# rgl-epfl/large-steps-pytorch

Measured on AMD Instinct MI355X. Metric: from_differential_solves_per_sec, higher is better.
Workload: dtype f32; 1 GPU; cfg4_plane1m: 1000x1000 plane, V=1000000, nnz(M)=6992002, M=I+50*L_uniform, u=M v, k=3, factor once (not timed), re-solve timed; method=nested-dissection, device=AMD Radeon Graphics

## Files before the change

### large-steps-pytorch_amd/csrc/direct.hip

```cpp
#include "common.h"
#include <vector>
#include <chrono>
#include <algorithm>
#include <atomic>
#include <string.h>
#include <memory>
#include <mutex>

namespace ls {

struct alignas(64) Tile {
    int store;
    int row0, s, b, own_start, bnd_off, front_off;
    int leaf;
    int pfront_off, cix;
    int forward;
    int arity;
    long long finv_off, w_off;
};

static_assert(sizeof(Tile) == 64, "Tile layout");
__device__ __forceinline__ Tile load_tile(const Tile* __restrict__ tiles, int idx) {
    const int lane = threadIdx.x & 63;
    const int w = lane < 16 ? reinterpret_cast<const int*>(tiles)[(size_t)idx * 16 + lane] : 0;
// ... 902 lines not shown
                    it.s = n.s; it.b = n.b; it.own_start = n.own_start; it.bnd_off = n.bnd_off; it.front_off = n.front_off;
                    it.pfront_off = n.pfront_off; it.cix = n.cix; it.flags = n.flags | (lv > root ? NODE_UPC : 0); it.finv_off = n.finv_off; it.w_off = n.w_off;
                    it.spb_off = n.spb_off; it.sps_off = n.sps_off; it.nparts = 1;
                    if (n.flags & NODE_SPARSE) {
                        items.push_back(it);
                        leaf_need = std::max(leaf_need, std::max(tri_cap, (4 * n.b + 3) & ~3) + 256);
                        continue;
                    }
                    if (n.s == 0 && n.b == 0) continue;
                    const int rows = up ? n.b : n.s, L = up ? ((n.s + 3) & ~3) : ((n.s + 3) & ~3) + ((n.b + 3) & ~3);
                    int nparts = 1;
                    if (!sparse && base < waves) nparts = std::max(1, std::min(waves / std::max(base, 1), L / 16));
                    for (int r = 0; r < std::max(rows, 1); r += WAVE)
                        for (int pt = 0; pt < nparts; ++pt) {
                            it.row0 = r; it.r0 = (int)((int64_t)(L / 4) * pt / nparts) * 4; it.r1 = (int)((int64_t)(L / 4) * (pt + 1) / nparts) * 4;
                            it.part = pt; it.nparts = nparts;
                            items.push_back(it);
                            vec_need = std::max(vec_need, 4 * (it.r1 - it.r0 + 32));
                        }
                    if (nparts > 1) { if (up) g.up_split |= 1u << ph; else g.down_split |= 1u << ph; }
                }
                if (all_sparse) { if (up) g.up_leaf |= 1u << ph; else g.down_leaf |= 1u << ph; }
                else if (sparse) return 0;
                const int n_items = (int)items.size() - off[ph];
                if (((up ? g.up_split : g.down_split) >> ph) & 1u) pbuf_need = std::max(pbuf_need, div_up(n_items, waves) * 256);
            }
            off[H] = (int)items.size();
        }
    }
    vec_floats = (vec_need + 3) & ~3;
    return (size_t)std::max(vec_floats + pbuf_need, leaf_need);
}


static size_t direct_tier_lds(int levels, int arity, const int* s, const int* b, const int* own_start, int tier_levels, bool sparse_leaves, int waves) {
    std::vector<int64_t> level_off((size_t)levels + 1);
    int64_t cnt = 1, off = 1;
    for (int lv = 0; lv <= levels; ++lv) { level_off[lv] = off; off += cnt; cnt *= arity; }
    const int64_t n_nodes = level_off[levels] - 1;
    std::vector<NodeD> nd((size_t)n_nodes + 1);
    memset(nd.data(), 0, nd.size() * sizeof(NodeD));
    const int root = levels - tier_levels;
    for (int lv = root; lv < levels; ++lv)
        for (int64_t i = level_off[lv]; i < level_off[lv + 1]; ++i) {
            NodeD& q = nd[(size_t)i];
            q.s = s[i]; q.b = b[i]; q.own_start = own_start[i];
            const bool sparse = sparse_leaves && lv == levels - 1 && q.s >= 1;
            q.flags = (lv + 1 >= levels ? NODE_LEAF : 0) | (sparse ? NODE_SPARSE : NODE_QUAD);
        }
    std::vector<TierItem> items;
    std::vector<TierWG> wgs;
    int vec = 0, tri = 0;
    const size_t region = plan_tier(nd, level_off, levels, arity, root, 0, level_off[root + 1] - level_off[root], items, wgs, vec, tri, waves);
    return region ? ((region + 3) & ~(size_t)3) * sizeof(float) * waves : 0;
}

bool direct_tier_fits(int levels, int arity, const int* s, const int* b, const int* own_start, int tier_levels, bool sparse_leaves, int waves) {
    if (tier_levels <= 0) return true;
    if (tier_levels > levels || tier_levels > TIER_MAX_H) return false;
    const size_t bytes = direct_tier_lds(levels, arity, s, b, own_start, tier_levels, sparse_leaves, waves);
    return bytes && bytes <= (size_t)(waves == TIER_WAVES_FULL ? TIER_LDS_FULL : TIER_LDS);
}

extern "C" int ls_direct_tier_lds_bytes(int levels, int arity, const int32_t* h_s, const int32_t* h_b, const int32_t* h_own_start, int tier_levels,
                                        int sparse_leaves, int waves, size_t* h_bytes) {
    LS_REQUIRE(h_s && h_b && h_own_start && h_bytes && levels >= 1 && levels <= 30 && (arity == 2 || arity == 4 || arity == 8) &&
               tier_levels >= 1 && tier_levels <= levels && tier_levels <= TIER_MAX_H && (waves == TIER_WAVES || waves == TIER_WAVES_WIDE || waves == TIER_WAVES_FULL),
               LS_E_INVALID, "ls_direct_tier_lds_bytes: bad argument (1 <= tier_levels <= min(levels, %d); waves 4, 8 or 16)", TIER_MAX_H);
    *h_bytes = direct_tier_lds(levels, arity, h_s, h_b, h_own_start, tier_levels, sparse_leaves != 0, waves);
    return LS_OK;
}

bool direct_tier_full16(int64_t V, int arity, int levels, int tier_levels, int shard_count, int tier_waves) {
    if (tier_waves == TIER_WAVES_FULL) return tier_levels >= 2;
    if (tier_waves == TIER_WAVES || tier_waves == TIER_WAVES_WIDE) return false;
    return shard_count <= 1 && arity == 4 && levels >= 8 && V >= 800000 && tier_levels == levels - 4 && tier_levels <= TIER_MAX_H;
}


namespace {
struct CreatePlan {
    int levels = 0, arity = 0, cut = 0;
    int64_t sub_lo = 0, sub_hi = 1;
    std::vector<int64_t> level_off;
    std::vector<NodeD> nd;
    std::vector<int> parent;
    std::vector<unsigned char> mask;
    std::vector<TierItem> items;
    std::vector<TierWG> wgs;
    std::vector<int> pull;
    std::vector<Tile> tiles;
    std::vector<PackedTile> ptiles;
    int64_t span(int from, int to) const { int64_t s = 1; for (int t = from; t < to; ++t) s *= arity; return s; }
    bool active(int64_t i, int lv) const {
        if (lv < cut) return true;
        int64_t q = i - level_off[lv];
        for (int t = cut; t < lv; ++t) q /= arity;
        return q >= sub_lo && q < sub_hi;
    }
};

int read_nodes(const ls_direct_arrays* A, CreatePlan& T, ls_direct* d) {
    const int levels = T.levels, n_nodes = d->n_nodes;
    T.nd.assign((size_t)n_nodes + 1, NodeD());
    T.parent.assign((size_t)n_nodes + 1, 0);
    d->lvl_up.assign((size_t)levels, 0); d->lvl_down.assign((size_t)levels, 0); d->lvl_rows.assign((size_t)levels, 0); d->lvl_bnd.assign((size_t)levels, 0);
    int64_t fe = 0, fe_up = 0, fe_down = 0;
// ... 27 lines not shown
    }
    fe += 2 * A->n_sp_ent + A->n_sp_ptr;
    fe_up += A->n_sp_ent + A->n_sp_ptr / 2; fe_down += A->n_sp_ent + A->n_sp_ptr - A->n_sp_ptr / 2;
    d->lvl_up[(size_t)levels - 1] += A->n_sp_ent + A->n_sp_ptr / 2; d->lvl_down[(size_t)levels - 1] += A->n_sp_ent + A->n_sp_ptr - A->n_sp_ptr / 2;
    d->factor_entries = fe; d->words_up = fe_up; d->words_down = fe_down;
    {
        const double mb = 4e-6 * (double)fe;
        d->nt_rule[0] = d->nt_levels = mb > 256.0;
        d->nt_rule[1] = d->nt_tier = mb > 400.0;
    }
    for (int lv = 1; lv < levels; ++lv)
        for (int64_t i = T.level_off[lv]; i < T.level_off[lv + 1]; ++i) {
            const NodeD &n = T.nd[i], &p = T.nd[T.parent[i]];
            for (int k = 0; k < n.b; ++k) {
                const int pp = A->h_ppos[n.bnd_off + k];
                if (pp < 0 || pp >= p.s + p.b) {
                    set_error("ls_direct_create: ppos out of range at node %lld", (long long)i);
                    return LS_E_INVALID;
                }
                T.mask[(size_t)p.front_off + pp] |= (unsigned char)(1u << n.cix);
            }
        }
    return LS_OK;
}

int choose_tier(CreatePlan& T, const int32_t* h_ppos, int tier_waves, const NdEnv& env, ls_direct* d) {
    const int levels = T.levels;
    int root = levels;
    for (int lv = levels - 1; lv >= 0; --lv) {
        bool tiered = false, plain = false;
        for (int64_t i = T.level_off[lv]; i < T.level_off[lv + 1]; ++i) {
            if (T.nd[i].s == 0 && T.nd[i].b == 0) continue;
            if (T.nd[i].flags & (NODE_SPARSE | NODE_QUAD)) tiered = true; else plain = true;
        }
        if (tiered && plain) { set_error("ls_direct_create: level %d mixes tier-layout and plain nodes", lv); return LS_E_INVALID; }
        if (plain) break;
        if (tiered && root != lv + 1) { set_error("ls_direct_create: tier-layout levels must be the deepest ones"); return LS_E_INVALID; }
        if (tiered) root = lv;
    }
    for (int lv = 0; lv < root; ++lv)
        for (int64_t i = T.level_off[lv]; i < T.level_off[lv + 1]; ++i)
            if (T.nd[i].flags & (NODE_SPARSE | NODE_QUAD)) { set_error("ls_direct_create: tier-layout node above the tier"); return LS_E_INVALID; }
    d->tier_root = levels;
    if (root == levels) return LS_OK;
    const int H = levels - root;
    if (T.cut > root) { set_error("ls_direct_create: %d ranks need a cut below the tier's root level (tree too small)", d->shard_count); return LS_E_INVALID; }
    const int64_t span = T.span(T.cut, root), q_lo = T.sub_lo * span, q_hi = T.sub_hi * span;
    size_t region = 0;
    auto take_if_fits = [&](int waves, int budget) {
        std::vector<TierItem> items;
        std::vector<TierWG> wgs;
        int vec = 0, tri = 0;
        const size_t r = plan_tier(T.nd, T.level_off, levels, T.arity, root, q_lo, q_hi, items, wgs, vec, tri, waves);
        if (!r || ((r + 3) & ~(size_t)3) * sizeof(float) * waves > (size_t)budget) return;
        T.items.swap(items); T.wgs.swap(wgs); d->tier_vec = vec; d->tier_tri = tri; region = r; d->tier_waves = waves;
    };
    if (H <= TIER_MAX_H && direct_tier_full16(d->V, T.arity, levels, H, d->shard_count, tier_waves > 0 ? tier_waves : env.tier_waves.value_or(0)))
        take_if_fits(TIER_WAVES_FULL, TIER_LDS_FULL);
    if (!region) {
        region = H <= TIER_MAX_H ? plan_tier(T.nd, T.level_off, levels, T.arity, root, q_lo, q_hi, T.items, T.wgs, d->tier_vec, d->tier_tri) : 0;
        if (!region || region * sizeof(float) * TIER_WAVES > TIER_LDS) {
            set_error("ls_direct_create: a tier of %d levels does not fit the kernel (LDS per wave: %zu floats)", H, region);
            return LS_E_WORKSPACE;
        }
        if (H >= 2 && (int)T.wgs.size() <= 768 && (tier_waves > 0 ? tier_waves : env.tier_waves.value_or(TIER_WAVES_WIDE)) == TIER_WAVES_WIDE)
            take_if_fits(TIER_WAVES_WIDE, TIER_LDS_WIDE);
    }
    d->tier_root = root; d->tier_phases = H; d->tier_wgs = (int)T.wgs.size(); d->tier_region = (int)((region + 3) & ~(size_t)3);
    d->pull_base = T.nd[T.level_off[root]].front_off;
    T.pull.assign((size_t)std::max<int64_t>(0, T.nd[T.level_off[levels - 1]].front_off - d->pull_base) * T.arity, -1);
    for (int lv = root + 1; lv < levels; ++lv)
        for (int64_t i = T.level_off[lv]; i < T.level_off[lv + 1]; ++i) {
            const NodeD& n = T.nd[i];
            for (int k = 0; k < n.b; ++k) T.pull[(size_t)(n.pfront_off - d->pull_base + h_ppos[n.bnd_off + k]) * T.arity + n.cix] = n.bnd_off + k;
        }
    return LS_OK;
}

size_t plan_level(CreatePlan& T, int lv, int long_up, const NdEnv& env, int kmax, LevelPlan& p) {
    std::vector<Tile>& tiles = T.tiles;
    int64_t a0 = T.level_off[lv], a1 = T.level_off[lv + 1];
    if (lv >= T.cut) { const int64_t span = T.span(T.cut, lv); a0 = T.level_off[lv] + T.sub_lo * span; a1 = T.level_off[lv] + T.sub_hi * span; }
    auto tile_of = [&](int64_t i, int r, int forward) {
        const NodeD& n = T.nd[i];
        Tile t;
        t.store = 0; t.row0 = r; t.s = n.s; t.b = n.b; t.own_start = n.own_start; t.bnd_off = n.bnd_off; t.front_off = n.front_off;
        t.leaf = lv + 1 >= T.levels; t.pfront_off = n.pfront_off; t.cix = n.cix;
        t.forward = forward; t.arity = T.arity; t.finv_off = n.finv_off; t.w_off = n.w_off;
        return t;
    };
    int red_up = 0, red_down = 0;
    for (int64_t i = a0; i < a1; ++i) {
        p.s_cap = std::max(p.s_cap, T.nd[i].s); p.b_cap = std::max(p.b_cap, T.nd[i].b);
        red_up = std::max(red_up, T.nd[i].s); red_down = std::max(red_down, T.nd[i].s + T.nd[i].b);
    }
    p.up_b = red_up >= long_up; p.down_b = red_down >= env.long_red;
    const int up_bw = std::min(ND_BW, red_up >= 1400 ? 8 : 4), down_bw = std::min(ND_BW, red_down >= 1400 ? 8 : 4);
    p.up_nw = p.up_b ? up_bw : pick_nw(red_up, 32); p.down_nw = p.down_b ? down_bw : pick_nw(red_down, env.steps);
    int64_t rows_up = 0, rows_down = 0;
    for (int64_t i = a0; i < a1; ++i) { rows_up += T.nd[i].b; rows_down += T.nd[i].s; }
    auto pick_chunks = [&](int64_t rows, int bw) {
        int c = 4;
        while (c > 1 && rows / (ND_ROWS * bw * c) < 500) --c;
        return c;
    };
    p.up_chunks = pick_chunks(rows_up, up_bw);
    p.down_chunks = pick_chunks(rows_down, down_bw);
    const int up_rows = p.up_b ? ND_ROWS * up_bw * p.up_chunks : WAVE, down_rows = p.down_b ? ND_ROWS * down_bw * p.down_chunks : WAVE;
    const size_t up_s_bytes = ((size_t)p.s_cap * p.b_cap + (size_t)p.s_cap * kmax) * sizeof(float);
    p.up_s = p.b_cap <= 256 && p.s_cap <= 256 && up_s_bytes <= 40 * 1024 && !env.no_small;
    if (p.up_s) { p.up_b = 0; p.up_nw = std::max(1, div_up(p.b_cap, WAVE)); }
    p.up_p = !env.no_pack && p.b_cap <= WAVE && p.s_cap <= 256 && lv > 0;
    p.down_p = !env.no_pack && p.s_cap <= WAVE / 2;
    auto pack_level = [&](bool up_sweep, int& first, int& count, int& lds_rows_s, int& lds_rows_b) {
// ... 218 lines not shown
#define LS_OPTIN(KK)                                                                                                                \
        (const void*)k_nd_up<KK, false>, (const void*)k_nd_down<KK, false>, (const void*)k_nd_up_b<KK, false>,                      \
        (const void*)k_nd_down_b<KK, false>, (const void*)k_nd_up<KK, true>, (const void*)k_nd_down<KK, true>,                      \
        (const void*)k_nd_up_b<KK, true>, (const void*)k_nd_down_b<KK, true>, (const void*)k_nd_up_s<KK>,
        LS_OPTIN(1) LS_OPTIN(2) LS_OPTIN(3) LS_OPTIN(4)
#undef LS_OPTIN
#define LS_OPTIN(KK)                                                                                                                \
        (const void*)k_nd_tier<KK, true, TIER_WAVES, false>, (const void*)k_nd_tier<KK, false, TIER_WAVES, false>,                  \
        (const void*)k_nd_tier<KK, true, TIER_WAVES, true>, (const void*)k_nd_tier<KK, false, TIER_WAVES, true>,                    \
        (const void*)k_nd_tier<KK, true, TIER_WAVES_WIDE, false>, (const void*)k_nd_tier<KK, false, TIER_WAVES_WIDE, false>,        \
        (const void*)k_nd_tier<KK, true, TIER_WAVES_FULL, false>, (const void*)k_nd_tier<KK, false, TIER_WAVES_FULL, false>,        \
        (const void*)k_nd_tier<KK, true, TIER_WAVES_FULL, true>, (const void*)k_nd_tier<KK, false, TIER_WAVES_FULL, true>,
        LS_OPTIN(1) LS_OPTIN(2) LS_OPTIN(3) LS_OPTIN(4)
#undef LS_OPTIN
    };
    for (const void* k : kernels) (void)hipFuncSetAttribute(k, hipFuncAttributeMaxDynamicSharedMemorySize, LDS_OPTIN);
    lap("kernel attributes set");
    *out = d.release();
    return LS_OK;
}

extern "C" int ls_direct_destroy(ls_direct* d) {
    if (!d) return LS_OK;
    DeviceGuard g(d->device);
    if (d->busy) (void)hipEventDestroy(d->busy);
    if (!d->tables.empty()) (void)hipDeviceSynchronize();
    for (const auto& t : d->tables)
        if (!ls::pool_give(d->device, t.first, t.second)) (void)hipFree(t.first);
    ls::refactor_state_free(d->refac);
    for (hipEvent_t e : d->ev) (void)hipEventDestroy(e);
#ifdef LS_TIER_STAMPS
    if (d->stamps) (void)hipFree(d->stamps);
#endif
    for (hipEvent_t e : d->lev) (void)hipEventDestroy(e);
    delete d;
    return LS_OK;
}

template <int K>
static int direct_solve_k(ls_direct* d, const float* b, float* x, hipStream_t st, int part, float* exchange) {
    const int top = d->tier_root - 1;
    TierArgs ta;
    ta.items = d->d_items; ta.wgs = d->d_wgs; ta.perm = d->perm; ta.mask = d->mask; ta.ppos = d->ppos;
    ta.pull = d->pull ? d->pull - (size_t)d->pull_base * d->arity : nullptr; ta.push_ptr = d->push_ptr; ta.push_tgt = d->push_tgt; ta.u4 = d->u4; ta.d4 = d->d4; ta.tri = d->tri;
    ta.sp_ptr = d->sp_ptr; ta.sp_ent = d->sp_ent; ta.bprime = d->bp; ta.braw = d->braw; ta.slots = d->slots; ta.xb = d->xb;
    ta.arity = d->arity; ta.phases = d->tier_phases; ta.region_floats = d->tier_region; ta.vec_floats = d->tier_vec;
    ta.upper_lo = d->upper_lo; ta.upper_hi = (int)d->V;
#ifdef LS_TIER_STAMPS
    const size_t stamp_n = (size_t)d->tier_wgs * d->tier_waves * TIER_STAMP_SLOTS;
    if (d->profile == 2 && !d->stamps && stamp_n) LS_HIP(hipMalloc((void**)&d->stamps, 2 * stamp_n * sizeof(long long)));
    if (d->profile == 2 && d->stamps) LS_HIP(hipMemsetAsync(d->stamps, 0, 2 * stamp_n * sizeof(long long), st));
    ta.stamps = d->profile == 2 ? d->stamps : nullptr;
#endif
    const size_t tier_lds = (size_t)d->tier_region * d->tier_waves * sizeof(float);
    const bool nt_tier = d->nt_tier && d->tier_waves != TIER_WAVES_WIDE, nt = d->nt_levels;
    int n_mark = 0;
    auto mark = [&](int lo, int hi, int sweep) -> hipError_t {
        if (d->profile != 3) return hipSuccess;
        while ((int)d->lev.size() <= n_mark + 1) { hipEvent_t e; const hipError_t r = hipEventCreate(&e); if (r != hipSuccess) return r; d->lev.push_back(e); }
        if ((int)d->lmeta.size() <= n_mark) d->lmeta.resize((size_t)n_mark + 1);
        d->lmeta[(size_t)n_mark] = {lo, hi, sweep};
        return hipEventRecord(d->lev[(size_t)n_mark++], st);
    };
    auto mark_end = [&]() -> hipError_t {
        if (d->profile != 3) return hipSuccess;
        hipError_t r = hipEventRecord(d->lev[(size_t)n_mark], st);
        if (r == hipSuccess) r = hipStreamSynchronize(st);
        d->launch_ms.assign((size_t)n_mark, 0.0);
        d->lmeta.resize((size_t)n_mark);
        for (int i = 0; i < n_mark && r == hipSuccess; ++i) { float ms = 0; r = hipEventElapsedTime(&ms, d->lev[(size_t)i], d->lev[(size_t)i + 1]); d->launch_ms[(size_t)i] = ms; }
        return r;
    };
    const size_t exch_off = (size_t)d->exch_f0 * d->arity * K, exch_n = (size_t)(d->exch_f1 - d->exch_f0) * d->arity * K;
    if (part != 1) {
    if (d->profile) LS_HIP(hipEventRecord(d->ev[0], st));
    if (part == 0 && exch_n) LS_HIP(hipMemsetAsync(d->slots + exch_off, 0, exch_n * sizeof(float), st));
    if (d->tier_wgs) {
        LS_HIP(mark(d->tier_root, d->levels - 1, 0));
        if (d->tier_waves == TIER_WAVES_FULL && nt_tier) hipLaunchKernelGGL((k_nd_tier<K, true, TIER_WAVES_FULL, true>), dim3(d->tier_wgs), dim3(WAVE * TIER_WAVES_FULL), tier_lds, st, ta, b, x, d->tier_tri);
        else if (d->tier_waves == TIER_WAVES_FULL) hipLaunchKernelGGL((k_nd_tier<K, true, TIER_WAVES_FULL, false>), dim3(d->tier_wgs), dim3(WAVE * TIER_WAVES_FULL), tier_lds, st, ta, b, x, d->tier_tri);
        else if (d->tier_waves == TIER_WAVES_WIDE) hipLaunchKernelGGL((k_nd_tier<K, true, TIER_WAVES_WIDE, false>), dim3(d->tier_wgs), dim3(WAVE * TIER_WAVES_WIDE), tier_lds, st, ta, b, x, d->tier_tri);
        else if (nt_tier) hipLaunchKernelGGL((k_nd_tier<K, true, TIER_WAVES, true>), dim3(d->tier_wgs), dim3(WAVE * TIER_WAVES), tier_lds, st, ta, b, x, d->tier_tri);
        else hipLaunchKernelGGL((k_nd_tier<K, true, TIER_WAVES, false>), dim3(d->tier_wgs), dim3(WAVE * TIER_WAVES), tier_lds, st, ta, b, x, d->tier_tri);
    }
    }
    if (part == 1 && exch_n && exchange != d->slots + exch_off)
        LS_HIP(hipMemcpyAsync(d->slots + exch_off, exchange, exch_n * sizeof(float), hipMemcpyDeviceToDevice, st));
    const int* up_perm = d->tier_wgs ? nullptr : d->perm;
    const float* up_b = d->tier_wgs ? d->braw : b;
    const bool fuse_root = top >= 0 && !d->plan[0].down_p;
    const RootFill rf = fuse_root ? RootFill{up_perm, d->mask, d->slots, up_b} : RootFill{nullptr, nullptr, nullptr, nullptr};
    for (int lv = (part == 1 ? std::min(top, d->cut - 1) : top); lv >= (part == 0 ? d->cut : 0); --lv) {
        const LevelPlan& p = d->plan[lv];
        if (!(p.up_p ? p.up_p_tiles : p.up_tiles)) continue;
        if (lv == 0 && fuse_root) continue;
        LS_HIP(mark(lv, lv, 0));
        if (p.up_p)
            hipLaunchKernelGGL(k_nd_up_p<K>, dim3(p.up_p_tiles), dim3(WAVE), (size_t)std::max(p.up_p_lds, 1) * K * sizeof(float), st,
                               d->ptiles + p.up_p_first, up_perm, d->mask, d->ppos, d->wf, up_b, d->bp, d->slots);
        else if (p.up_s)
            hipLaunchKernelGGL(k_nd_up_s<K>, dim3(p.up_tiles), dim3(WAVE * p.up_nw), ((size_t)p.s_cap * p.b_cap + (size_t)p.s_cap * K) * sizeof(float), st,
                               d->tiles + p.up_first, up_perm, d->mask, d->ppos, d->wf, up_b, d->bp, d->slots, p.s_cap, p.b_cap);
        else if (p.up_b)
            hipLaunchKernelGGL((nt ? k_nd_up_b<K, true> : k_nd_up_b<K, false>), dim3(p.up_tiles), dim3(WAVE * p.up_nw), ((size_t)p.s_cap * K + 16) * sizeof(float), st,
                               d->tiles + p.up_first, up_perm, d->mask, d->ppos, d->wb, up_b, d->bp, d->slots, p.s_cap, p.up_chunks);
        else
            hipLaunchKernelGGL((nt ? k_nd_up<K, true> : k_nd_up<K, false>), dim3(p.up_tiles), dim3(WAVE * p.up_nw),
// ... 280 lines not shown
```

### large-steps-pytorch_amd/csrc/nd_tier.h

```cpp
#pragma once

namespace ls {

constexpr int TIER_MAX_H = 6;
constexpr int TIER_WAVES = 4;
constexpr int TIER_WAVES_WIDE = 8;
constexpr int TIER_WAVES_FULL = 16;
constexpr int TIER_LDS_FULL = 160 * 1024;
constexpr int TIER_LDS = 150 * 1024;
constexpr int TIER_LDS_WIDE = 80 * 1024;
constexpr int LEVEL_LDS = 150 * 1024;
constexpr int LDS_OPTIN = 160 * 1024;
constexpr int TIER_TRI4 = 9;
constexpr int TIER_SPE = 4;

enum : int { NODE_LEAF = 1, NODE_SPARSE = 2, NODE_QUAD = 4, NODE_UPC = 8 };

struct SpEnt { float val; int idx; };

struct NodeD {
    int s, b, own_start, bnd_off, front_off, pfront_off, cix, flags;
    long long finv_off, w_off;
    int spb_off, sps_off;
};

struct alignas(32) TierItem {
    int s, b, own_start, bnd_off, front_off, pfront_off, cix, flags;
    long long finv_off, w_off;
    int spb_off, sps_off;
    int row0, r0, r1, part, nparts, pad0, pad1, pad2;
};
static_assert(sizeof(TierItem) == 96, "TierItem layout");

struct alignas(64) TierWG {
    int up_off[TIER_MAX_H + 1];
    int down_off[TIER_MAX_H + 1];
    unsigned up_split, down_split;
    unsigned up_leaf, down_leaf;
    int n_dense, pad;
    int dense_rng[2 * TIER_MAX_H];
};
static_assert(sizeof(TierWG) == 128, "TierWG layout (read as 32 dwords)");

struct TierArgs {
    const TierItem* items;
    const TierWG* wgs;
    const int* perm;
    const unsigned char* mask;
    const int* ppos;
    const int* pull;
    const int* push_ptr;
    const int* push_tgt;
    const float* u4;
    const float* d4;
    const float* tri;
    const int* sp_ptr;
    const SpEnt* sp_ent;
    float* bprime;
    int upper_lo, upper_hi;
    float* braw;
    float* slots;
    float* xb;
    int arity, phases, region_floats, vec_floats;
#ifdef LS_TIER_STAMPS
    long long* stamps;
#endif
};
// ... 249 lines not shown
                const SpEnt z = a.sp_ent[p];
#pragma unroll
                for (int q = 0; q < K; ++q) u[q] = fmaf(z.val, yv[z.idx * 4 + q], u[q]);
            }
            const size_t dst = upc ? (size_t)(n.bnd_off + i) * K : ((size_t)(n.pfront_off + pp) * a.arity + n.cix) * K;
            float* out = upc ? a.xb : a.slots;
#pragma unroll
            for (int q = 0; q < K; ++q) out[dst + q] = u[q];
        }
    }
    wave_lds_sync();
}

template <int K>
__device__ __forceinline__ void leaf_down_head(const TierArgs& a, const TierItem& n, const LeafIdx& ix, const float (&xv)[K],
                                               const SpEnt (&e)[TIER_SPE], float* region, float (&t)[K]) {
    const int lane = threadIdx.x & 63, b = n.b;
    float* xbv = region;
    if (lane < b) {
#pragma unroll
        for (int q = 0; q < K; ++q) xbv[lane * 4 + q] = xv[q];
    }
    for (int i = lane + 64; i < b; i += 64) {
#pragma unroll
        for (int q = 0; q < K; ++q) xbv[i * 4 + q] = a.xb[(size_t)(n.bnd_off + i) * K + q];
    }
    wave_lds_sync();
    sparse_row<K>(a, ix, e, xbv, t);
    wave_lds_sync();
}

template <int K>
__device__ __forceinline__ void leaf_down_vec(const TierItem& n, const float (&t)[K], float* region, int tri_floats) {
    const int lane = threadIdx.x & 63;
    float4 w = make_float4(0.f, 0.f, 0.f, 0.f);
    if (lane < n.s) { w.x = t[0]; if (K > 1) w.y = t[K > 1 ? 1 : 0]; if (K > 2) w.z = t[K > 2 ? 2 : 0]; if (K > 3) w.w = t[K > 3 ? 3 : 0]; }
    reinterpret_cast<float4*>(region + tri_floats)[lane] = w;
}

template <int K>
__device__ __forceinline__ void leaf_down_tail(const TierItem& n, const LeafIdx& ix, const float (&yj)[K], float* __restrict__ x_out,
                                               float* region, int tri_floats) {
    const int lane = threadIdx.x & 63, s = n.s;
    float z[K];
    tri_matvec<K>(region, region + tri_floats, s, lane, z);
    if (lane < s) {
#pragma unroll
        for (int q = 0; q < K; ++q) x_out[(size_t)ix.g * K + q] = yj[q] - z[q];
    }
    wave_lds_sync();
}

template <int K, bool UP, int W, bool NT>
__device__ __forceinline__ void leaf_phase(const TierArgs& a, int k0, int k1, const float* __restrict__ b_in, float* __restrict__ x_out,
                                           float* region, int tri_floats, long long* stamp_base) {
    const int lane = threadIdx.x & 63;
    int leaf_no = 0;
    (void)leaf_no; (void)stamp_base;
    if (k0 >= k1) return;
    constexpr int S = W;
    TierItem it = rec_unpack(rec_load(a.items, k0, lane));
    int rec_n = k0 + S < k1 ? rec_load(a.items, k0 + S, lane) : 0;
    LeafIdx ix;
    leaf_idx<UP>(a, it, lane, ix);
    for (int k = k0; k < k1; k += S) {
        float v[K];
        SpEnt e[TIER_SPE];
        float t[K];
        {
            LeafDat<K> d;
            leaf_dat<K, UP, NT>(a, it, ix, b_in, lane, d);
            if (!UP) leaf_down_head<K>(a, it, ix, d.xv, d.e, region, t);
            tri_stage<K>(d, it.s, lane, region);
#pragma unroll
            for (int q = 0; q < K; ++q) v[q] = d.v[q];
#pragma unroll
            for (int u = 0; u < TIER_SPE; ++u) e[u] = d.e[u];
        }
        if (!UP) leaf_down_vec<K>(it, t, region, tri_floats);
        wave_lds_sync();
        const bool more = k + S < k1;
        TierItem it_n = it;
        LeafIdx ix_n = ix;
        if (more) { it_n = rec_unpack(rec_n); leaf_idx<UP>(a, it_n, lane, ix_n); }
        rec_n = k + 2 * S < k1 ? rec_load(a.items, k + 2 * S, lane) : 0;
        if (UP) leaf_up_compute<K>(a, it, ix, v, e, region, tri_floats);
        else leaf_down_tail<K>(it, ix, v, x_out, region, tri_floats);
        if (leaf_no < 8) LS_STAMP(16 + leaf_no);
        ++leaf_no;
        it = it_n; ix = ix_n;
    }
}

#ifndef LS_TIER_Q
#define LS_TIER_Q 4
#endif
constexpr int TIER_Q = LS_TIER_Q;

template <bool NT>
__device__ __forceinline__ void tier_prefetch(const float4* __restrict__ col, size_t rows, int q0, int q1, float4 (&cur)[TIER_Q]) {
#pragma unroll
    for (int e = 0; e < TIER_Q; ++e) cur[e] = (q0 + e < q1) ? ld_stream4<NT>(col + (size_t)(q0 + e) * rows) : make_float4(0.f, 0.f, 0.f, 0.f);
}

__device__ __forceinline__ void tier_mv16(float v16, const float4& a, const float4& b, const float4& c, const float4& d, int n, f32x4& acc) {
    acc = mv_step<0>(v16, a.x, acc); acc = mv_step<1>(v16, a.y, acc); acc = mv_step<2>(v16, a.z, acc); acc = mv_step<3>(v16, a.w, acc);
    if (n > 1) { acc = mv_step<4>(v16, b.x, acc); acc = mv_step<5>(v16, b.y, acc); acc = mv_step<6>(v16, b.z, acc); acc = mv_step<7>(v16, b.w, acc); }
    if (n > 2) { acc = mv_step<8>(v16, c.x, acc); acc = mv_step<9>(v16, c.y, acc); acc = mv_step<10>(v16, c.z, acc); acc = mv_step<11>(v16, c.w, acc); }
    if (n > 3) { acc = mv_step<12>(v16, d.x, acc); acc = mv_step<13>(v16, d.y, acc); acc = mv_step<14>(v16, d.z, acc); acc = mv_step<15>(v16, d.w, acc); }
}

__device__ __forceinline__ void tier_mv_batch(const float* sv4, int base, int q, int q1, const float4 (&c)[TIER_Q], f32x4& acc) {
    const int lane = threadIdx.x & 63;
    const float4 z = make_float4(0.f, 0.f, 0.f, 0.f);
    if (TIER_Q == 2) tier_mv16(sv4[(4 * q - base) * 4 + lane], c[0], c[1], z, z, min(2, q1 - q), acc);
    if (TIER_Q >= 4) tier_mv16(sv4[(4 * q - base) * 4 + lane], c[0], c[1], c[TIER_Q >= 4 ? 2 : 0], c[TIER_Q >= 4 ? 3 : 0], q1 - q, acc);
    if (TIER_Q >= 8 && q + 4 < q1) tier_mv16(sv4[(4 * q + 16 - base) * 4 + lane], c[TIER_Q >= 8 ? 4 : 0], c[TIER_Q >= 8 ? 5 : 0],
                                             c[TIER_Q >= 8 ? 6 : 0], c[TIER_Q >= 8 ? 7 : 0], q1 - q - 4, acc);
}
template <bool NT>
__device__ __forceinline__ void tier_dot(const float4* __restrict__ col, size_t rows, int q0, int q1, const float* sv4, int base,
                                         float4 (&A)[TIER_Q], float4 (&B)[TIER_Q], f32x4& acc) {
    for (int q = q0; q < q1; q += 2 * TIER_Q) {
        tier_mv_batch(sv4, base, q, q1, A, acc);
        tier_prefetch<NT>(col, rows, q + 2 * TIER_Q, q1, A);
        if (q + TIER_Q < q1) tier_mv_batch(sv4, base, q + TIER_Q, q1, B, acc);
        tier_prefetch<NT>(col, rows, q + 3 * TIER_Q, q1, B);
    }
}

template <int K>
__device__ __forceinline__ void node_up_finish(const TierArgs& a, const TierItem& n, int i, int pp, const float (&acc)[K]) {
    if (i >= n.b || n.pfront_off < 0) return;
    if (n.flags & NODE_UPC) {
#pragma unroll
        for (int q = 0; q < K; ++q) a.xb[(size_t)(n.bnd_off + i) * K + q] = acc[q];
        return;
    }
    const size_t dst = ((size_t)(n.pfront_off + pp) * a.arity + n.cix) * K;
#pragma unroll
    for (int q = 0; q < K; ++q) a.slots[dst + q] = acc[q];
}

template <int K>
// ... 181 lines not shown
    wave_lds_sync();
#pragma unroll
    for (int c = 0; c < 4; ++c) P.plb[c] = (it.nparts == 1 && P.plo[0] + c < P.plo[1]) ? a.push_tgt[P.plo[0] + c] : -1;
    f32x4 a4 = {0.f, 0.f, 0.f, 0.f};
    tier_dot<NT>(col, (size_t)s, it.r0 >> 2, it.r1 >> 2, sv4, it.r0, P.cur, B, a4);
    float acc[K];
#pragma unroll
    for (int q = 0; q < K; ++q) acc[q] = a4[q];
    if (it.nparts == 1) node_down_store<K>(a, it, P.idx, P.plo[0], P.plo[1], P.plb, x_out, acc);
    else {
#pragma unroll
        for (int q = 0; q < K; ++q) pbuf[lane * 4 + q] = acc[q];
    }
#pragma unroll
    for (int c = 0; c < 2; ++c) {
        if (ftg[c] >= 0) {
#pragma unroll
            for (int q = 0; q < K; ++q) a.xb[(size_t)ftg[c] * K + q] = fv[q];
        }
    }
    if (fw && P.fw1 - P.fw0 > 2) push_down<K>(a.push_tgt, P.fw0 + 2, P.fw1, a.xb, fv);
    if (!(it.flags & NODE_LEAF)) {
        for (int i = f0 + 64 + lane; i < f1; i += 64) {
            const size_t f = (size_t)(it.front_off + s + i);
            const int p0 = a.push_ptr[f], p1 = a.push_ptr[f + 1];
            float v[K];
#pragma unroll
            for (int q = 0; q < K; ++q) v[q] = a.xb[(size_t)(it.bnd_off + i) * K + q];
            push_down<K>(a.push_tgt, p0, p1, a.xb, v);
        }
    }
    wave_lds_sync();
}

template <int K, bool UP, int W, bool NT>
__global__ __launch_bounds__(64 * W, 16 / W) void k_nd_tier(TierArgs a, const float* __restrict__ b_in, float* __restrict__ x_out,
                                                              int tri_floats) {
    extern __shared__ __attribute__((aligned(16))) float sm[];
    const int wave = __builtin_amdgcn_readfirstlane(threadIdx.x >> 6), lane = threadIdx.x & 63;
    float* region = sm + (size_t)wave * a.region_floats;
    for (int i = lane; 4 * i < a.region_floats; i += 64) reinterpret_cast<float4*>(region)[i] = make_float4(0.f, 0.f, 0.f, 0.f);
    wave_lds_sync();
    const int n_wg = (int)gridDim.x;
    const int sub = __builtin_expect((n_wg & 7) == 0, 1) ? (int)(blockIdx.x & 7) * (n_wg >> 3) + (int)(blockIdx.x >> 3) : (int)blockIdx.x;
#ifdef LS_TIER_STAMPS
    long long* stamp_base = a.stamps ? a.stamps + ((size_t)sub * W + wave) * TIER_STAMP_SLOTS : nullptr;
#else
    long long* stamp_base = nullptr;
#endif
    LS_STAMP(0);
    const int hdr = lane < 32 ? reinterpret_cast<const int*>(a.wgs + sub)[lane] : 0;
    const int obase = UP ? 0 : TIER_MAX_H + 1;
    const unsigned split = (unsigned)rl(hdr, UP ? 14 : 15), leafy = (unsigned)rl(hdr, UP ? 16 : 17);
    if (UP) {
        const int n_dense = rl(hdr, 18);
        for (int r = threadIdx.x; r < n_dense; r += blockDim.x) {
            int o = r, start = 0;
#pragma unroll
            for (int t = 0; t < TIER_MAX_H; ++t) {
                const int cnt = rl(hdr, 20 + 2 * t + 1);
                const bool here = o >= 0 && o < cnt;
                start = here ? rl(hdr, 20 + 2 * t) + o : start;
                o = here ? -1 : o - cnt;
            }
            const size_t g = (size_t)a.perm[start];
#pragma unroll
            for (int q = 0; q < K; ++q) a.braw[(size_t)start * K + q] = b_in[g * K + q];
        }
        for (int r = a.upper_lo + blockIdx.x * blockDim.x + threadIdx.x; r < a.upper_hi; r += gridDim.x * blockDim.x) {
            const size_t g = (size_t)a.perm[r];
#pragma unroll
            for (int q = 0; q < K; ++q) a.braw[(size_t)r * K + q] = b_in[g * K + q];
        }
    }
    LS_STAMP(1);
    DensePre<K> pre;
#pragma unroll
    for (int e = 0; e < TIER_Q; ++e) pre.cur[e] = make_float4(0.f, 0.f, 0.f, 0.f);
#pragma unroll
    for (int q = 0; q < K; ++q) pre.v[q] = 0.0f;
    pre.idx = 0; pre.fw0 = 1; pre.fw1 = 0;
#pragma unroll
    for (int c = 0; c < 4; ++c) { pre.plo[c] = -1; pre.plb[c] = -1; }
    TierItem it_pre = rec_unpack(0);
    bool pre_valid = false;
    for (int ph = 0; ph < a.phases; ++ph) {
        const int i0 = rl(hdr, obase + ph), i1 = rl(hdr, obase + ph + 1);
        int rec_nx = 0;
        bool has_nx = false;
        if (ph + 1 < a.phases && !((leafy >> (ph + 1)) & 1u)) {
            const int j0 = rl(hdr, obase + ph + 1) + wave;
            has_nx = j0 < rl(hdr, obase + ph + 2);
            if (has_nx) rec_nx = rec_load(a.items, j0, lane);
        }
        if ((leafy >> ph) & 1u) {
            leaf_phase<K, UP, W, NT>(a, i0 + wave, i1, b_in, x_out, region, tri_floats, stamp_base);
        } else {
            int rec = (!pre_valid && i0 + wave < i1) ? rec_load(a.items, i0 + wave, lane) : 0;
            int head_k = -1, head_idx = 0, head_p0 = 0, head_p1 = 0, head_flags = 0;
            for (int k = i0 + wave; k < i1; k += W) {
                const int rec_next = k + W < i1 ? rec_load(a.items, k + W, lane) : 0;
                const bool first = k == i0 + wave && pre_valid;
                const TierItem it = first ? it_pre : rec_unpack(rec);
                rec = rec_next;
                float* pbuf = region + a.vec_floats + ((k - i0) / W) * 256;
                if (!first) { if (UP) node_up_pre<K, NT>(a, it, pre); else node_down_pre<K, NT>(a, it, pre); }
                if (UP) node_up<K, NT>(a, it, pre, b_in, region, pbuf);
                else node_down<K, NT>(a, it, pre, x_out, region, pbuf);
                if (it.nparts > 1 && it.part == 0) {
                    head_k = k; head_idx = pre.idx; head_p0 = pre.plo[0]; head_p1 = pre.plo[1]; head_flags = it.flags;
                }
            }
            if ((split >> ph) & 1u) {
                const int rec_head = head_k >= 0 ? rec_load(a.items, head_k, lane) : 0;
                int head_tg[4];
#pragma unroll
                for (int c = 0; c < 4; ++c) head_tg[c] = (!UP && head_k >= 0 && head_p0 + c < head_p1 && !(head_flags & NODE_LEAF)) ? a.push_tgt[head_p0 + c] : -1;
                __syncthreads();
                for (int k = i0 + wave; k < i1; k += W) {
                    const bool mine = k == head_k;
                    const TierItem it = rec_unpack(mine ? rec_head : rec_load(a.items, k, lane));
                    if (it.nparts == 1 || it.part != 0) continue;
                    float acc[K];
#pragma unroll
                    for (int q = 0; q < K; ++q) acc[q] = 0.0f;
                    for (int p = 0; p < it.nparts; ++p) {
                        const int kp = k + p - i0;
                        const float* pb = sm + (size_t)(kp % W) * a.region_floats + a.vec_floats + (kp / W) * 256;
#pragma unroll
                        for (int q = 0; q < K; ++q) acc[q] += pb[lane * 4 + q];
                    }
                    if (UP) {
                        const int i = it.row0 + lane;
                        const int pp = mine ? head_idx : ((i < it.b && it.pfront_off >= 0 && !(it.flags & NODE_UPC)) ? a.ppos[it.bnd_off + i] : 0);
                        node_up_finish<K>(a, it, i, pp, acc);
                    } else if (mine) {
                        node_down_store<K>(a, it, head_idx, head_p0, head_p1, head_tg, x_out, acc);
                    }
                    else node_down_finish<K>(a, it, x_out, acc);
                }
            }
        }
        if (ph < 6) { LS_STAMP(2 + 2 * ph); LS_STAMP_VAL(24 + ph, (i1 - i0 - wave + W - 1) / W); }
        pre_valid = has_nx;
        it_pre = rec_unpack(rec_nx);
        if (pre_valid) {
            if (UP) node_up_pre<K, NT>(a, it_pre, pre); else node_down_pre<K, NT>(a, it_pre, pre);
        } else {
#pragma unroll
            for (int e = 0; e < TIER_Q; ++e) pre.cur[e] = make_float4(0.f, 0.f, 0.f, 0.f);
#pragma unroll
            for (int q = 0; q < K; ++q) pre.v[q] = 0.0f;
            pre.idx = 0; pre.fw0 = 1; pre.fw1 = 0;
#pragma unroll
            for (int c = 0; c < 4; ++c) { pre.plo[c] = -1; pre.plb[c] = -1; }
        }
        __syncthreads();
        if (ph < 6) LS_STAMP(3 + 2 * ph);
    }
}

}
```

Measured before the change: 5197 solves/s.

## Dynamically schedule down-sweep leaf items via LDS ticket counter

In the down sweep, leaf items within a workgroup are now handed out by an LDS atomic ticket instead of a static stride of W per wave, which balances uneven leaf costs across waves. The first leaf item of a leafy phase is also preloaded and indexed ahead of time, during dense setup or the previous phase. The LDS budget grows by a 16-byte ticket slot and all fit checks are updated to include it. The cost is an extra atomic and a lane broadcast per leaf, plus a dependency on the drawn ticket before the next record can be prefetched.

```diff
diff --git a/large-steps-pytorch_amd/csrc/direct.hip b/large-steps-pytorch_amd/csrc/direct.hip
--- a/large-steps-pytorch_amd/csrc/direct.hip
+++ b/large-steps-pytorch_amd/csrc/direct.hip
@@ -978,7 +978,7 @@
     std::vector<TierWG> wgs;
     int vec = 0, tri = 0;
     const size_t region = plan_tier(nd, level_off, levels, arity, root, 0, level_off[root + 1] - level_off[root], items, wgs, vec, tri, waves);
-    return region ? ((region + 3) & ~(size_t)3) * sizeof(float) * waves : 0;
+    return region ? ((region + 3) & ~(size_t)3) * sizeof(float) * waves + TIER_LDS_TICKET : 0;
 }
 
 bool direct_tier_fits(int levels, int arity, const int* s, const int* b, const int* own_start, int tier_levels, bool sparse_leaves, int waves) {
@@ -1112,14 +1112,14 @@
         std::vector<TierWG> wgs;
         int vec = 0, tri = 0;
         const size_t r = plan_tier(T.nd, T.level_off, levels, T.arity, root, q_lo, q_hi, items, wgs, vec, tri, waves);
-        if (!r || ((r + 3) & ~(size_t)3) * sizeof(float) * waves > (size_t)budget) return;
+        if (!r || ((r + 3) & ~(size_t)3) * sizeof(float) * waves + TIER_LDS_TICKET > (size_t)budget) return;
         T.items.swap(items); T.wgs.swap(wgs); d->tier_vec = vec; d->tier_tri = tri; region = r; d->tier_waves = waves;
     };
     if (H <= TIER_MAX_H && direct_tier_full16(d->V, T.arity, levels, H, d->shard_count, tier_waves > 0 ? tier_waves : env.tier_waves.value_or(0)))
         take_if_fits(TIER_WAVES_FULL, TIER_LDS_FULL);
     if (!region) {
         region = H <= TIER_MAX_H ? plan_tier(T.nd, T.level_off, levels, T.arity, root, q_lo, q_hi, T.items, T.wgs, d->tier_vec, d->tier_tri) : 0;
-        if (!region || region * sizeof(float) * TIER_WAVES > TIER_LDS) {
+        if (!region || ((region + 3) & ~(size_t)3) * sizeof(float) * TIER_WAVES + TIER_LDS_TICKET > TIER_LDS) {
             set_error("ls_direct_create: a tier of %d levels does not fit the kernel (LDS per wave: %zu floats)", H, region);
             return LS_E_WORKSPACE;
         }
@@ -1444,7 +1444,7 @@
     if (d->profile == 2 && d->stamps) LS_HIP(hipMemsetAsync(d->stamps, 0, 2 * stamp_n * sizeof(long long), st));
     ta.stamps = d->profile == 2 ? d->stamps : nullptr;
 #endif
-    const size_t tier_lds = (size_t)d->tier_region * d->tier_waves * sizeof(float);
+    const size_t tier_lds = (size_t)d->tier_region * d->tier_waves * sizeof(float) + TIER_LDS_TICKET;
     const bool nt_tier = d->nt_tier && d->tier_waves != TIER_WAVES_WIDE, nt = d->nt_levels;
     int n_mark = 0;
     auto mark = [&](int lo, int hi, int sweep) -> hipError_t {
diff --git a/large-steps-pytorch_amd/csrc/nd_tier.h b/large-steps-pytorch_amd/csrc/nd_tier.h
--- a/large-steps-pytorch_amd/csrc/nd_tier.h
+++ b/large-steps-pytorch_amd/csrc/nd_tier.h
@@ -13,6 +13,7 @@
 constexpr int LDS_OPTIN = 160 * 1024;
 constexpr int TIER_TRI4 = 9;
 constexpr int TIER_SPE = 4;
+constexpr int TIER_LDS_TICKET = 16;
 
 enum : int { NODE_LEAF = 1, NODE_SPARSE = 2, NODE_QUAD = 4, NODE_UPC = 8 };
 
@@ -368,24 +369,32 @@
 }
 
 template <int K, bool UP, int W, bool NT>
-__device__ __forceinline__ void leaf_phase(const TierArgs& a, int k0, int k1, const float* __restrict__ b_in, float* __restrict__ x_out,
-                                           float* region, int tri_floats, long long* stamp_base) {
+__device__ __forceinline__ int leaf_phase(const TierArgs& a, int i0, int n, int wave, TierItem it, LeafIdx ix, int* ticket,
+                                          const float* __restrict__ b_in, float* __restrict__ x_out,
+                                          float* region, int tri_floats, long long* stamp_base) {
+#ifndef LS_TICKET
+#define LS_TICKET 1
+#endif
+    constexpr bool TICKET = !UP && LS_TICKET;
     const int lane = threadIdx.x & 63;
     int leaf_no = 0;
-    (void)leaf_no; (void)stamp_base;
-    if (k0 >= k1) return;
-    constexpr int S = W;
-    TierItem it = rec_unpack(rec_load(a.items, k0, lane));
-    int rec_n = k0 + S < k1 ? rec_load(a.items, k0 + S, lane) : 0;
-    LeafIdx ix;
-    leaf_idx<UP>(a, it, lane, ix);
-    for (int k = k0; k < k1; k += S) {
+    (void)stamp_base;
+    if (wave >= n) return 0;
+    int k_n = wave + W;
+    int rec_n = (!TICKET && k_n < n) ? rec_load(a.items, i0 + k_n, lane) : 0;
+    for (;;) {
+        int drawn = 0;
+        if (TICKET && lane == 0) drawn = (int)__builtin_amdgcn_atomic_inc32(reinterpret_cast<unsigned*>(ticket), 0x7fffffffu, __ATOMIC_RELAXED, "workgroup");
         float v[K];
         SpEnt e[TIER_SPE];
         float t[K];
         {
             LeafDat<K> d;
             leaf_dat<K, UP, NT>(a, it, ix, b_in, lane, d);
+            if (TICKET) {
+                k_n = rl(drawn, 0);
+                rec_n = k_n < n ? rec_load(a.items, i0 + k_n, lane) : 0;
+            }
             if (!UP) leaf_down_head<K>(a, it, ix, d.xv, d.e, region, t);
             tri_stage<K>(d, it.s, lane, region);
 #pragma unroll
@@ -395,17 +404,19 @@
         }
         if (!UP) leaf_down_vec<K>(it, t, region, tri_floats);
         wave_lds_sync();
-        const bool more = k + S < k1;
+        const bool more = k_n < n;
         TierItem it_n = it;
         LeafIdx ix_n = ix;
         if (more) { it_n = rec_unpack(rec_n); leaf_idx<UP>(a, it_n, lane, ix_n); }
-        rec_n = k + 2 * S < k1 ? rec_load(a.items, k + 2 * S, lane) : 0;
+        if (!TICKET) { k_n += W; rec_n = k_n < n ? rec_load(a.items, i0 + k_n, lane) : 0; }
         if (UP) leaf_up_compute<K>(a, it, ix, v, e, region, tri_floats);
         else leaf_down_tail<K>(it, ix, v, x_out, region, tri_floats);
         if (leaf_no < 8) LS_STAMP(16 + leaf_no);
         ++leaf_no;
+        if (!more) break;
         it = it_n; ix = ix_n;
     }
+    return leaf_no;
 }
 
 #ifndef LS_TIER_Q
@@ -693,6 +704,13 @@
     const int hdr = lane < 32 ? reinterpret_cast<const int*>(a.wgs + sub)[lane] : 0;
     const int obase = UP ? 0 : TIER_MAX_H + 1;
     const unsigned split = (unsigned)rl(hdr, UP ? 14 : 15), leafy = (unsigned)rl(hdr, UP ? 16 : 17);
+    int* ticket = reinterpret_cast<int*>(sm + (size_t)W * a.region_floats);
+    if (!UP) {
+        if (threadIdx.x == 0) *ticket = W;
+        if (leafy & 1u) __syncthreads();
+    }
+    bool lead_valid = (leafy & 1u) && rl(hdr, obase) + wave < rl(hdr, obase + 1);
+    const int rec_lead = lead_valid ? rec_load(a.items, rl(hdr, obase) + wave, lane) : 0;
     if (UP) {
         const int n_dense = rl(hdr, 18);
         for (int r = threadIdx.x; r < n_dense; r += blockDim.x) {
@@ -714,6 +732,9 @@
             for (int q = 0; q < K; ++q) a.braw[(size_t)r * K + q] = b_in[g * K + q];
         }
     }
+    TierItem it_pre = rec_unpack(rec_lead);
+    LeafIdx ix_pre = {0, 0, 0, 0};
+    if (lead_valid) leaf_idx<UP>(a, it_pre, lane, ix_pre);
     LS_STAMP(1);
     DensePre<K> pre;
 #pragma unroll
@@ -723,19 +744,21 @@
     pre.idx = 0; pre.fw0 = 1; pre.fw1 = 0;
 #pragma unroll
     for (int c = 0; c < 4; ++c) { pre.plo[c] = -1; pre.plb[c] = -1; }
-    TierItem it_pre = rec_unpack(0);
     bool pre_valid = false;
     for (int ph = 0; ph < a.phases; ++ph) {
         const int i0 = rl(hdr, obase + ph), i1 = rl(hdr, obase + ph + 1);
         int rec_nx = 0;
         bool has_nx = false;
-        if (ph + 1 < a.phases && !((leafy >> (ph + 1)) & 1u)) {
+        const bool nx_leafy = ph + 1 < a.phases && ((leafy >> (ph + 1)) & 1u);
+        if (ph + 1 < a.phases) {
             const int j0 = rl(hdr, obase + ph + 1) + wave;
             has_nx = j0 < rl(hdr, obase + ph + 2);
             if (has_nx) rec_nx = rec_load(a.items, j0, lane);
         }
+        int ran = (i1 - i0 - wave + W - 1) / W;
+        (void)ran;
         if ((leafy >> ph) & 1u) {
-            leaf_phase<K, UP, W, NT>(a, i0 + wave, i1, b_in, x_out, region, tri_floats, stamp_base);
+            ran = leaf_phase<K, UP, W, NT>(a, i0, i1 - i0, wave, it_pre, ix_pre, ticket, b_in, x_out, region, tri_floats, stamp_base);
         } else {
             int rec = (!pre_valid && i0 + wave < i1) ? rec_load(a.items, i0 + wave, lane) : 0;
             int head_k = -1, head_idx = 0, head_p0 = 0, head_p1 = 0, head_flags = 0;
@@ -782,9 +805,12 @@
                 }
             }
         }
-        if (ph < 6) { LS_STAMP(2 + 2 * ph); LS_STAMP_VAL(24 + ph, (i1 - i0 - wave + W - 1) / W); }
-        pre_valid = has_nx;
+        if (ph < 6) { LS_STAMP(2 + 2 * ph); LS_STAMP_VAL(24 + ph, ran); }
+        pre_valid = has_nx && !nx_leafy;
+        lead_valid = has_nx && nx_leafy;
         it_pre = rec_unpack(rec_nx);
+        ix_pre = LeafIdx{0, 0, 0, 0};
+        if (lead_valid) leaf_idx<UP>(a, it_pre, lane, ix_pre);
         if (pre_valid) {
             if (UP) node_up_pre<K, NT>(a, it_pre, pre); else node_down_pre<K, NT>(a, it_pre, pre);
         } else {
```

Result: no change. 5214 solves/s (median of 6 runs) (+0.3%).
